# NilFoundation/vote-saver-protocol

Hardware: AMD Instinct MI355X
Metric: G1 MSM points/sec at 2^20 (Groth16 prover hot path) (higher is better)
Workload: dtype u32; 1 GPU; 2^20-point BLS12-381 G1 Pippenger MSM per GPU, PLAIN bases k_i*G (no table of window multiples; the library's 28-bit-limb copy keeps phi(P) = (beta x, y) beside every P for the endomorphism split), uniform scalars, bases and scalars resident in HBM; N ranks = one 2^20*N-point MSM sharded by contiguous chunk, RCCL all-gather of Jacobian partial sums + fold; points_per_gpu=1048576, window_bits=16, windows=8, endomorphism_split=True, msms_in_flight=4, bases_precomputed_window_multiples=False, bases_memory_bytes_per_point=352

## Files before the change

### vote_saver_protocol_amd/csrc/common.h

```cpp
#pragma once
#include <hip/hip_runtime.h>
#include <stdint.h>
#include <stdio.h>
#include <string.h>
#include <functional>
#include <initializer_list>
#include <map>
#include <string>
#include <vector>

#include "../../include/vsp.h"
#include <atomic>
#include <mutex>
#include <thread>
#include "curve.h"
#include "point_decode.h"
#include "saver_ct.h"
#include "saver_rerand.h"

struct vsp_ctx;
namespace vsp {

struct Affine28; struct Affine28x2;
template <int N> struct Group;
// ... 62 lines not shown

struct MsmGeom {
    unsigned c;
    unsigned W;
    unsigned B;
    unsigned q0, q1, q2;
    unsigned T;
    size_t n;
    size_t G;
    unsigned Wr;
    unsigned single;
    uint32_t idx_stride, idx_first;
    unsigned sbits;
    unsigned lb;
    unsigned fold;
    unsigned bd;
    unsigned K, Wk;
    size_t kstride;
};
struct MsmPre { size_t stride; size_t first; unsigned c; const void *table28; bool glv; };

struct MsmWork {
    static constexpr size_t PINNED_BYTES = 256 * 1024;
    bool inited = false, own_stream = false, active = false, empty = false;
    bool dimbits = false;
    hipStream_t stream = nullptr;
    hipStream_t own = nullptr;
    hipEvent_t ev0 = nullptr, ev1 = nullptr, done = nullptr, plan_ready = nullptr;
    DevBuf cnt, off, cursor, nsub, suboff, blocksum, sorted, heavy, counters, digits, blockhist, partbucket, perm, sizehist;
    DevBuf buckets, partials, dims, winres, medium, redo;
    DevBuf buckets28, partials28;
    DevBuf pairs_a, pairs_b, ms_h1, ms_h1s, ms_h2, ms_h2s;
    DevBuf tmp_sorted, tmp_lo, off_hi, cnt_hi;
    DevBuf glv_scalars;
    bool glv = false;
    void *h_pinned = nullptr;
    size_t pinned_cap = 0;
    static constexpr unsigned REC_RING = 4;
    void *h_rec = nullptr; hipEvent_t rec_ev[REC_RING] = {nullptr, nullptr, nullptr, nullptr}; unsigned rec_idx = 0;
    void *h_census = nullptr;
    hipEvent_t census_done = nullptr;
    bool census_pending = false; size_t census_n = 0; const void *census_scalars = nullptr;
    bool check_pending = false;
    size_t neff_cache_n = 0, neff_cache = 0;
    MsmGeom g;
    size_t n = 0, n_eff = 0;
};
static constexpr unsigned VSP_MSM_SLOTS = 6;
struct MsmTuning { long window_bits = 0, split = 0, dimbits = -1; };
struct MsmRequest {
    const void *bases = nullptr;
    const Fr *scalars = nullptr;
    size_t n = 0;
    int plan_from = -1;
    bool dense = false;
    bool plan_only = false;
    const MsmPre *pre = nullptr;
    const void *table28 = nullptr;
    bool glv = false;
    unsigned batch = 0;
    size_t stride = 0;
    const MsmTuning *tuning = nullptr;
    MsmRequest(const Fr *scalars_ = nullptr, size_t n_ = 0) : scalars(scalars_), n(n_) {}
};
struct MsmLaunch {
    MsmRequest rq;
    hipStream_t st;
    const MsmWork *plan_from;
    const void *table28;
    const Fr *scalars; size_t n;
    long sort_mode;
    MsmTuning tune;
    bool fused_split, fused_scans, dimbits;
    size_t M, Smax;
    unsigned per_w, nblk, gblk, ablk;
};
static constexpr unsigned MSM_THREADS = 256;
static constexpr unsigned SZ_BINS = 1024;
__device__ __forceinline__ uint32_t part_len(uint32_t s, uint32_t parts) { return (s + parts - 1) / parts; }

enum NttPath { NTT_AUTO, NTT_FR29, NTT_FR32 };
struct NttRequest {
    const Fr *in[3] = {nullptr, nullptr, nullptr};
    Fr *out[3] = {nullptr, nullptr, nullptr};
    unsigned count = 1;
    size_t in_stride = 0, out_stride = 0;
    const Fr *fuse_b = nullptr, *fuse_c = nullptr;
    unsigned log_m = 0;
    int inverse = 0;
    const uint64_t *coset_g = nullptr;
    const HFr *extra_scale = nullptr;
    NttPath path = NTT_AUTO;
    NttRequest(Fr *d_a, unsigned log_m_, int inverse_ = 0, const uint64_t *coset_g_ = nullptr, const HFr *extra_scale_ = nullptr)
        : log_m(log_m_), inverse(inverse_), coset_g(coset_g_), extra_scale(extra_scale_) { in[0] = d_a; out[0] = d_a; }
};

}

struct vsp_ctx {
    int device = 0;
    hipStream_t stream = nullptr;
    hipStream_t own_stream = nullptr;
    hipStream_t prove_streams[2] = {nullptr, nullptr};
    hipEvent_t ev0 = nullptr, ev1 = nullptr, ev_aux = nullptr;
    std::string err;
    std::map<std::string, double> stats;
// ... 418 lines not shown
```

### vote_saver_protocol_amd/csrc/msm_impl.inc

```
#include "common.h"
#include "lane_view.h"
#include "fp28.h"
#if VSP_MSM_GROUP == 1
#include "accum28_asm_gfx950.h"
#endif


namespace vsp {
namespace {

#if VSP_MSM_GROUP == 1
static constexpr uint32_t GLV_BETA_MONT[12] = {0x8671f071u, 0xcd03c9e4u, 0x1fcda5d2u, 0x5dab2246u, 0xd3851b95u, 0x587042afu, 0x01bacb9eu, 0x8eb60ebeu, 0x83d050d2u, 0x03f97d6eu, 0x54638741u, 0x18f02065u};
#else
static constexpr uint32_t GLV_BETA_MONT[12] = {0x798a64e8u, 0x30f1361bu, 0x7ece5a2au, 0xf3b8ddabu, 0xc61577f7u, 0x16a8ca3au, 0x74fd029bu, 0xc26a2ff8u, 0x60701c6eu, 0x3636b766u, 0x241b6160u, 0x051ba4abu};
#endif
__device__ __forceinline__ Fp glv_beta() { Fp b; for (int i = 0; i < 12; i++) b.l[i] = GLV_BETA_MONT[i]; return b; }
__device__ __forceinline__ void glv_apply(Fp &x) { x = mul(x, glv_beta()); }
__device__ __forceinline__ void glv_apply(Fp2 &x) { Fp b = glv_beta(); x.c0 = mul(x.c0, b); x.c1 = mul(x.c1, b); }
__device__ __forceinline__ void glv_apply(Fp2L &x) { x.v = mul(x.v, glv_beta()); }

template <class F> struct AccumWaves { static constexpr unsigned W = 2; };
template <class F>
__device__ __forceinline__ XYZZ<typename LaneView<F>::E> accumulate_part(const Affine<F> *__restrict__ bases, const uint32_t *__restrict__ sorted, const uint32_t *__restrict__ off,
                                                const uint32_t *__restrict__ suboff, const uint32_t *__restrict__ part_bucket, uint32_t q,
// ... 750 lines not shown
    const long wide = opt(ctx, "msm_wide_windows", 1);
    if (c == 16 && wide && !glv && n >= ((size_t)1 << 20)) c = 17;
    if (c >= 16 && wide && n >= ((size_t)1 << 23)) {
        double best = 0; int bc = 16;
        for (int k = 16; k <= 23; k++) {
            const double W = glv ? (double)((128 + k - 1) / k) : (double)((255 % k == 0 ? 254 : 255) / k + 1);
            const double cost = (double)n * W * (k > 16 ? 0.87 : 1.0) + W * (double)((size_t)1 << (k - 1)) * 4.1;
            if (k == 16 || cost < best) { best = cost; bc = k; }
        }
        c = bc;
    }
    return (unsigned)c;
}

#if VSP_MSM_GROUP == 1
using F28 = Fp28; using Row28 = Affine28;
#else
using F28 = Fp2x28; using Row28 = Affine28x2;
#endif

template <class F> static int msm_geometry(vsp_ctx *ctx, MsmWork &wk, MsmLaunch &L, MsmGeom &g, size_t &n_eff) {
    const MsmPre *pre = L.rq.pre; const bool glv = L.rq.glv; const size_t n = L.rq.n; const unsigned batch = L.rq.batch;
    const uint32_t imul = glv ? 2u : 1u;
    n_eff = n;
    if (L.plan_from) {
        g = L.plan_from->g; n_eff = L.plan_from->n_eff;
        if (L.plan_from->n != n) return set_error(ctx, VSP_ERR_ARG, "msm: shared plan of a different size");
        if ((g.single != 0) != (pre != nullptr) || (pre && (g.idx_stride != pre->stride * imul || g.idx_first != pre->first * imul || g.c != pre->c)))
            return set_error(ctx, VSP_ERR_ARG, "msm: shared plan needs bases precomputed alike");
    } else {
        VSP_TRY(ensure_w(ctx, L.st, wk.counters, 64));
        wk.check_pending = false;
        if (!L.rq.dense) {
            if (!(wk.census_pending && wk.census_n == n && wk.census_scalars == (const void *)L.rq.scalars)) VSP_TRY(msm_census(ctx, wk, L.rq.scalars, n, nullptr, batch, L.rq.stride));
            wk.check_pending = true;
            if (n >= 4096) {
                if (wk.neff_cache_n == n && !opt(ctx, "msm_census_sync", 0)) n_eff = wk.neff_cache;
                else {
                    VSP_HIP(hipEventSynchronize(wk.census_done));
                    uint32_t h_cnt = *(volatile uint32_t *)wk.h_census / batch;
                    n_eff = h_cnt < 256 ? 256 : h_cnt;
                }
            }
        }
        wk.census_pending = false;
        if (glv) n_eff *= 2;
        g.c = pre ? pre->c : pick_window_bits(ctx, L.tune.window_bits, n_eff, glv);
        g.sbits = glv ? 128u : 255u;
        g.fold = (!glv && opt(ctx, "msm_fold", 1) && 255u % g.c == 0u) ? 1u : 0u;
        if (batch > 1 && g.c > 16) g.c = 16;
        if (batch > 1 && g.c < 7) g.c = 7;
        g.Wk = glv ? (128u + g.c - 1) / g.c : (g.fold ? 254u / g.c + 1 : g.sbits / g.c + 1);
        g.K = batch; g.kstride = batch > 1 ? L.rq.stride : 0;
        g.W = g.Wk * g.K;
        g.B = 1u << (g.c - 1);
        g.lb = g.c > 16 ? g.c - 16 : 0u;
        g.n = glv ? 2 * n : n;
        g.single = pre ? 1u : 0u; g.idx_stride = pre ? (uint32_t)(pre->stride * imul) : 0u; g.idx_first = pre ? (uint32_t)(pre->first * imul) : 0u;
        g.Wr = pre ? g.K : g.W;
        g.G = (size_t)g.Wr * g.B;
        const long t = L.tune.split;
        if (pre) {
            size_t est = n_eff * g.W / ((size_t)1 << 18);
            unsigned T = 16; while (T < est && T < (1u << 20)) T <<= 1;
            if (T >= 64) T = T / 8 * 7;
            g.T = t > 0 ? (unsigned)t : T;
            if ((size_t)g.Wk * pre->stride * imul >= ((size_t)1 << 31)) return set_error(ctx, VSP_ERR_UNSUPPORTED, "msm: precomputed table too large to index");
        } else {
            size_t mean = n_eff / g.B + 1;
            size_t T = mean * 4 < 128 ? 128 : mean * 4;
// ... 80 lines not shown
                           g.G, g.T, buckets28, partials28, redo + 1, redo);
        VSP_HIP(hipEventRecord(wk.ev1, st));
        hipLaunchKernelGGL(HIP_KERNEL_NAME(k_accum_redo<F>), dim3(L.ablk < 64 ? L.ablk : 64), dim3(MSM_THREADS), 0, st, bases, (const uint32_t *)pl->sorted.p,
                           (const uint32_t *)pl->off.p, (const uint32_t *)pl->suboff.p, (const uint32_t *)pl->partbucket.p, buckets, partials,
                           (const uint32_t *)(redo + 1), (const uint32_t *)redo, L.rq.glv, buckets28, partials28);
        VSP_LAUNCH_CHECK();
        return launch_tail<F28>(ctx, st, pl, g, L.dimbits, buckets28, partials28, (XYZZ<F28> *)wk.dims.p, winres, (XYZZ<F> *)wk.h_pinned);
    }
    VSP_HIP(hipEventRecord(wk.ev0, st));
    hipLaunchKernelGGL(HIP_KERNEL_NAME(k_accum<F>), dim3(L.ablk * LaneView<F>::LANES), dim3(MSM_THREADS), 0, st, bases, (const uint32_t *)pl->sorted.p,
                       (const uint32_t *)pl->off.p, (const uint32_t *)pl->suboff.p, (const uint32_t *)pl->perm.p, (const uint32_t *)pl->partbucket.p,
                       g.G, g.T, buckets, partials);
    VSP_HIP(hipEventRecord(wk.ev1, st));
    VSP_LAUNCH_CHECK();
    return launch_tail<F>(ctx, st, pl, g, L.dimbits, buckets, partials, (XYZZ<F> *)wk.dims.p, winres, (XYZZ<F> *)wk.h_pinned);
}

template <class F>
static int msm_launch(vsp_ctx *ctx, MsmWork &wk, const MsmRequest &rq, const MsmWork *plan_from) {
    const size_t n = rq.n;
    wk.active = false; wk.n = n;
    if (n == 0) { wk.active = true; wk.empty = true; wk.g.K = rq.batch ? rq.batch : 1; return VSP_OK; }
    wk.empty = false;
    const unsigned batch = rq.batch ? rq.batch : 1;
    if (batch > 1 && rq.plan_only) return set_error(ctx, VSP_ERR_UNSUPPORTED, "msm: a batch plans and accumulates in one launch");
    if (batch > 1 && plan_from && (plan_from->g.K != batch || plan_from->g.kstride != rq.stride || !plan_from->active || plan_from->empty))
        return set_error(ctx, VSP_ERR_ARG, "msm: shared plan of another batch");
    MsmLaunch L{};
    L.rq = rq; L.rq.batch = batch; L.st = wk.stream; L.scalars = rq.scalars; L.n = n;
    L.table28 = rq.pre ? rq.pre->table28 : rq.table28;
    L.rq.glv = rq.glv && (rq.pre ? rq.pre->glv && rq.pre->table28 : rq.table28 != nullptr);
    if (n >= ((size_t)1 << (L.rq.glv ? 30 : 31))) return set_error(ctx, VSP_ERR_UNSUPPORTED, "msm: n >= 2^31");
    L.plan_from = plan_from && plan_from->glv == L.rq.glv ? plan_from : nullptr;
    wk.glv = L.rq.glv;
    L.sort_mode = opt(ctx, "msm_sort", 0);
    L.tune = rq.tuning ? *rq.tuning : MsmTuning{opt(ctx, "msm_window_bits", 0), opt(ctx, "msm_split", 0), opt(ctx, "msm_dimbits", -1)};
    MsmGeom g; size_t n_eff = n;
    VSP_TRY(msm_geometry<F>(ctx, wk, L, g, n_eff));
    wk.g = g; wk.n_eff = n_eff;
    VSP_TRY(msm_split_scalars(ctx, wk, L, g));
    VSP_TRY(msm_buffers<F>(ctx, wk, L, g));
    if (L.plan_from) VSP_HIP(hipStreamWaitEvent(L.st, L.plan_from->plan_ready, 0));
    else { VSP_TRY(msm_digit_sort(ctx, wk, L, g)); VSP_TRY(msm_bucket_plan(ctx, wk, L, g)); }
    if (rq.plan_only) return VSP_OK;
    VSP_TRY(msm_accumulate<F>(ctx, wk, L, g));
    VSP_HIP(hipEventRecord(wk.done, L.st));
    wk.active = true;
    return VSP_OK;
}

template <class F, class HF> static void msm_fold(const MsmWork &wk, XYZZ<HF> *out);
template <class F, class HF>
static int msm_finish_wait(vsp_ctx *ctx, MsmWork &wk, unsigned out_count, bool *empty);
template <class F, class HF>
static int msm_finish(vsp_ctx *ctx, MsmWork &wk, XYZZ<HF> *out, unsigned out_count = 1) {
    for (unsigned k = 0; k < out_count; k++) out[k] = XYZZ<HF>::inf();
    bool empty = false;
    VSP_TRY((msm_finish_wait<F, HF>(ctx, wk, out_count, &empty)));
    if (!empty) msm_fold<F, HF>(wk, out);
    return VSP_OK;
}
template <class F, class HF>
static int msm_finish_wait(vsp_ctx *ctx, MsmWork &wk, unsigned out_count, bool *empty) {
    static_assert(sizeof(F) == sizeof(HF), "host/device field layouts must match");
    *empty = true;
    if (!wk.active) return set_error(ctx, VSP_ERR_ARG, "msm: finish without launch");
    wk.active = false;
    if (wk.empty) return VSP_OK;
    *empty = false;
    if (wk.g.K != out_count) return set_error(ctx, VSP_ERR_ARG, "msm: finish asks for another number of results than the launch's batch");
    VSP_HIP(hipEventSynchronize(wk.done));
    const MsmGeom &g = wk.g;
#ifdef VSP_DEBUG_DUMP
    if (const char *dir = getenv("VSP_DEBUG_DUMP_DIR")) {
        if (FILE *f = fopen((std::string(dir) + "/winres.bin").c_str(), "wb")) { fwrite(wk.h_pinned, 1, (size_t)g.Wr * (wk.dimbits ? DIMBITS_STRIDE : 4) * sizeof(XYZZ<HF>), f); fclose(f); }
        const unsigned per_w = dims_per_w(g);
        std::vector<char> hb(g.G * sizeof(XYZZ<F>)), hd((size_t)g.Wr * per_w * sizeof(XYZZ<F>));
        if (wk.buckets.p && wk.dims.p && hipMemcpy(hb.data(), wk.buckets.p, hb.size(), hipMemcpyDeviceToHost) == hipSuccess &&
            hipMemcpy(hd.data(), wk.dims.p, hd.size(), hipMemcpyDeviceToHost) == hipSuccess) {
            std::string d(dir);
            if (FILE *f = fopen((d + "/buckets.bin").c_str(), "wb")) { fwrite(hb.data(), 1, hb.size(), f); fclose(f); }
            if (FILE *f = fopen((d + "/dims.bin").c_str(), "wb")) { fwrite(hd.data(), 1, hd.size(), f); fclose(f); }
            if (FILE *f = fopen((d + "/geom.txt").c_str(), "w")) { fprintf(f, "%u %u %u %u %u %u %u %zu\n", g.c, g.W, g.Wr, g.B, g.q0, g.q1, g.q2, sizeof(XYZZ<F>)); fclose(f); }
        }
    }
#endif
    if (wk.check_pending) {
        wk.check_pending = false;
        VSP_HIP(hipEventSynchronize(wk.census_done));
        const volatile uint32_t *hc = (const volatile uint32_t *)wk.h_census;
        if (wk.n >= 4096) { const uint32_t c0 = hc[0] / (wk.g.K ? wk.g.K : 1u); wk.neff_cache_n = wk.n; wk.neff_cache = c0 < 256 ? 256 : c0; }
        if (hc[2]) return set_error(ctx, VSP_ERR_ARG, "msm: a scalar is not canonical (>= r)");
    }
    float ms = 0.f;
    if (hipEventElapsedTime(&ms, wk.ev0, wk.ev1) == hipSuccess) {
        ctx->stats["msm_accum_ms"] += ms;
        ctx->stats["msm_accum_launches"] += 1;
    }
    ctx->stats["msm_calls"] += 1;
    ctx->stats["msm_n_eff"] = (double)wk.n_eff;
    ctx->stats["msm_window_bits"] = g.c;
    ctx->stats["msm_windows"] = g.W;
    ctx->stats["msm_bucket_sets"] = g.Wr;
    ctx->stats["msm_split"] = g.T;
    ctx->stats["msm_endomorphism_split"] = wk.glv ? 1 : 0;
    if (opt(ctx, "msm_debug_counts", 0) && wk.counters.p && wk.suboff.p) {
        uint32_t c4[4] = {0, 0, 0, 0}, parts = 0;
        if (hipMemcpy(c4, wk.counters.p, sizeof c4, hipMemcpyDeviceToHost) == hipSuccess &&
            hipMemcpy(&parts, (const uint32_t *)wk.suboff.p + g.G, 4, hipMemcpyDeviceToHost) == hipSuccess) {
            ctx->stats["msm_heavy_buckets"] = c4[0]; ctx->stats["msm_medium_buckets"] = c4[2]; ctx->stats["msm_parts"] = parts;
            ctx->stats["msm_buckets"] = (double)g.G;
        }
    }
    return VSP_OK;
}
template <class F, class HF> static void msm_fold(const MsmWork &wk, XYZZ<HF> *out) {
    const MsmGeom &g = wk.g;
    const XYZZ<HF> *wr = (const XYZZ<HF> *)wk.h_pinned;
    const unsigned per = g.single ? 1u : (g.K > 1 ? g.Wk : g.Wr);
// ... 111 lines not shown
```

### vote_saver_protocol_amd/csrc/msm_sort.hip

```cpp
#include "common.h"

namespace vsp {
namespace {


__device__ __forceinline__ uint32_t scalar_bits(const uint32_t *k, unsigned pos, unsigned c) {
    unsigned limb = pos >> 5, sh = pos & 31;
    if (limb >= 8) return 0;
    uint64_t v = k[limb];
    if (limb + 1 < 8) v |= (uint64_t)k[limb + 1] << 32;
    return (uint32_t)(v >> sh) & ((1u << c) - 1u);
}

__device__ __forceinline__ uint32_t load_scalar(const Fr *scalars, size_t i, const MsmGeom &g, uint32_t (&k)[8]) {
    const uint32_t *p = scalars[i].l;
#pragma unroll
    for (int j = 0; j < 8; j++) k[j] = p[j];
    if (g.sbits == 128u) return k[7] >> 31;
    if (!g.fold) return 0u;
    uint32_t d[8], borrow = 0;
#pragma unroll
    for (int j = 0; j < 8; j++) {
        const uint64_t t = (uint64_t)FrP32::MOD[j] - k[j] - borrow;
        d[j] = (uint32_t)t; borrow = (uint32_t)(t >> 63);
// ... 150 lines not shown
    if (threadIdx.x == 0 && bad) atomicOr(&counters[3], 1u);
}

#ifndef VSP_CS_ATTR
#define VSP_CS_ATTR
#endif
#ifndef VSP_CS_UNROLL
#define VSP_CS_UNROLL
#endif
#ifndef VSP_CS_THREADS
#define VSP_CS_THREADS 1024
#endif
static constexpr unsigned CS_THREADS = VSP_CS_THREADS;
static constexpr unsigned CS_MLP = 8;
static constexpr uint16_t DIGIT_NONE = 0xFFFFu;

__global__ __launch_bounds__(256) void k_digits(const Fr *scalars, MsmGeom g, uint16_t *digits, uint8_t *flips) {
    size_t i = (size_t)blockIdx.x * blockDim.x + threadIdx.x;
    if (i >= g.n) return;
    const unsigned kb = blockIdx.y;
    scalars += (size_t)kb * g.kstride;
    uint32_t k[8];
    const uint32_t flip = load_scalar(scalars, i, g, k);
    uint32_t carry = 0;
    if (g.sbits == 128u || g.fold) flips[(size_t)kb * g.n + i] = (uint8_t)flip;
    for (unsigned w = 0; w < g.Wk; w++) {
        uint32_t raw = scalar_bits(k, w * g.c, g.c) + carry;
        uint32_t mag; uint32_t neg;
        if (raw > g.B) { mag = (1u << g.c) - raw; neg = 1; carry = 1; }
        else { mag = raw; neg = 0; carry = 0; }
        digits[(size_t)(kb * g.Wk + w) * g.n + i] = mag ? (uint16_t)((mag - 1) | (neg << 15)) : DIGIT_NONE;
    }
}
__global__ __launch_bounds__(256) void k_glv_digits(const Fr *scalars, size_t n_orig, MsmGeom g, uint16_t *digits, uint8_t *flips) {
    size_t i = (size_t)blockIdx.x * blockDim.x + threadIdx.x;
    if (i >= n_orig) return;
    const unsigned kb = blockIdx.y;
    scalars += (size_t)kb * g.kstride;
    flips += (size_t)kb * g.n;
    uint32_t k[8], m[2][8]; bool neg[2];
    load_scalar_words(scalars, i, k);
    {
        uint32_t m1[4], m2[4];
        glv_split_scalar(k, m1, neg[0], m2, neg[1]);
#pragma unroll
        for (int j = 0; j < 8; j++) { m[0][j] = j < 4 ? m1[j] : 0u; m[1][j] = j < 4 ? m2[j] : 0u; }
    }
    reinterpret_cast<uint16_t *>(flips)[i] = (uint16_t)((neg[0] ? 1u : 0u) | (neg[1] ? 0x100u : 0u));
    uint32_t carry[2] = {0, 0};
    uint32_t *d32 = reinterpret_cast<uint32_t *>(digits);
    for (unsigned w = 0; w < g.Wk; w++) {
        uint32_t pair = 0;
#pragma unroll
        for (int b = 0; b < 2; b++) {
            const uint32_t raw = scalar_bits(m[b], w * g.c, g.c) + carry[b];
            uint32_t mag, ng;
            if (raw > g.B) { mag = (1u << g.c) - raw; ng = 1; carry[b] = 1; }
            else { mag = raw; ng = 0; carry[b] = 0; }
            const uint32_t d = mag ? ((mag - 1) | (ng << 15)) : (uint32_t)DIGIT_NONE;
            pair |= d << (16 * b);
        }
        d32[((size_t)(kb * g.Wk + w) * g.n) / 2 + i] = pair;
    }
}

__global__ __launch_bounds__(256) void k_digits_wide(const Fr *scalars, MsmGeom g, uint16_t *hi, uint8_t *lo) {
    size_t i = (size_t)blockIdx.x * blockDim.x + threadIdx.x;
    if (i >= g.n) return;
    uint32_t k[8];
    const uint32_t flip = load_scalar(scalars, i, g, k);
    uint32_t carry = 0;
    for (unsigned w = 0; w < g.W; w++) {
        uint32_t raw = scalar_bits(k, w * g.c, g.c) + carry;
// ... 78 lines not shown
    for (size_t base = i0; base < i1; base += (size_t)CS_MLP * CS_THREADS) {
        uint16_t dd[CS_MLP]; uint8_t ff[CS_MLP];
#pragma unroll
        for (unsigned j = 0; j < CS_MLP; j++) {
            const size_t i = base + (size_t)j * CS_THREADS + threadIdx.x;
            dd[j] = i < i1 ? dw[i] : DIGIT_NONE;
            ff[j] = (use_flips && i < i1) ? flips[(size_t)(w / g.Wk) * g.n + i] : (uint8_t)0;
        }
#pragma unroll
        for (unsigned j = 0; j < CS_MLP; j++) {
            const size_t i = base + (size_t)j * CS_THREADS + threadIdx.x;
            const uint16_t d = dd[j];
            const bool valid = d != DIGIT_NONE;
            const uint32_t key = d & 0x7FFFu;
            const unsigned long long act = __ballot(valid);
            if (act) {
                const int lead = __ffsll((long long)act) - 1;
                const uint32_t lkey = (uint32_t)__shfl((int)key, lead, 64);
                const bool same = valid && key == lkey;
                const unsigned long long grp = __ballot(same);
                const unsigned lane = threadIdx.x & 63u;
                uint32_t pos = 0;
                if (same && (int)lane == lead) pos = atomicAdd(&lds_cur[lkey], (uint32_t)__popcll(grp));
                pos = (uint32_t)__shfl((int)pos, lead, 64) + (uint32_t)__popcll(grp & ((1ull << lane) - 1ull));
                if (valid && !same) pos = atomicAdd(&lds_cur[key], 1u);
                if (valid) {
                    uint32_t sign;
                    if (lo_in) { const uint8_t l = lo_in[(size_t)w * g.n + i]; sign = l >> 7; lo_out[pos] = l & 0x7Fu; }
                    else sign = (uint32_t)(d >> 15) ^ (uint32_t)ff[j];
                    sorted[pos] = entry_of(g, w, i) | (sign << 31);
                }
            }
        }
    }
}

__global__ __launch_bounds__(256) void k_segment_sort(const uint32_t *__restrict__ tmp_sorted, const uint8_t *__restrict__ tmp_lo, const uint32_t *__restrict__ off_hi,
                                                     size_t segments, unsigned lb, uint32_t *cnt, uint32_t *off, uint32_t *sorted) {
    __shared__ uint32_t sh[4][128];
    const unsigned wave = threadIdx.x >> 6, lane = threadIdx.x & 63u;
    uint32_t *c = sh[wave];
    const unsigned nb = 1u << lb;
    const unsigned long long below = (1ull << lane) - 1ull;
    for (size_t s = (size_t)blockIdx.x * 4 + wave; s < segments; s += (size_t)gridDim.x * 4) {
        const uint32_t a = off_hi[s], b = off_hi[s + 1];
        c[lane] = 0; c[lane + 64] = 0;
        __builtin_amdgcn_wave_barrier();
        for (uint32_t j0 = a; j0 < b; j0 += 64) {
            const uint32_t j = j0 + lane;
            const bool valid = j < b;
            const uint32_t l = valid ? tmp_lo[j] : 0u;
            unsigned long long peers = __ballot(valid);
            for (unsigned k = 0; k < lb; k++) { const bool bit = (l >> k) & 1u; const unsigned long long m = __ballot(valid && bit); peers &= bit ? m : ~m; }
            if (valid && (int)lane == __ffsll((long long)peers) - 1) atomicAdd(&c[l], (uint32_t)__popcll(peers));
        }
        __builtin_amdgcn_wave_barrier();
        const uint32_t c0 = c[lane], c1 = c[lane + 64];
        uint32_t i0 = c0, i1 = c1;
        for (int d = 1; d < 64; d <<= 1) { uint32_t x0 = __shfl_up(i0, d, 64), x1 = __shfl_up(i1, d, 64); if ((int)lane >= d) { i0 += x0; i1 += x1; } }
        const uint32_t tot0 = __shfl(i0, 63, 64);
        const uint32_t e0 = a + i0 - c0, e1 = a + tot0 + i1 - c1;
        const size_t g0 = (s << lb) + lane;
        if (lane < nb) { cnt[g0] = c0; off[g0] = e0; }
        if (lane + 64 < nb) { cnt[g0 + 64] = c1; off[g0 + 64] = e1; }
        __builtin_amdgcn_wave_barrier();
        c[lane] = e0; c[lane + 64] = e1;
// ... 540 lines not shown
    VSP_TRY(ensure_w(ctx, st, wk.off_hi, (gh.G + 1) * 4));
    VSP_TRY(ensure_w(ctx, st, wk.tmp_sorted, L.M * 4));
    VSP_TRY(ensure_w(ctx, st, wk.tmp_lo, L.M));
    uint16_t *hi = (uint16_t *)wk.digits.p; uint8_t *lo = (uint8_t *)(hi + (size_t)g.W * n);
    uint32_t *blockhist = (uint32_t *)wk.blockhist.p, *cnt_hi = (uint32_t *)wk.cnt_hi.p, *off_hi = (uint32_t *)wk.off_hi.p;
    const size_t lds_bytes = (size_t)gh.B * sizeof(uint32_t);
    VSP_TRY(lds_sort_attrs(ctx));
    hipLaunchKernelGGL(k_digits_wide, dim3(L.nblk), dim3(MSM_THREADS), 0, st, L.scalars, g, hi, lo);
    hipLaunchKernelGGL(k_count_lds, dim3(nchunks * g.W), dim3(CS_THREADS), lds_bytes, st, (const uint16_t *)hi, gh, nchunks, chunk_len, blockhist);
    hipLaunchKernelGGL(k_chunk_prefix, dim3((unsigned)((gh.G + MSM_THREADS - 1) / MSM_THREADS)), dim3(MSM_THREADS), 0, st, blockhist, g.single ? nchunks * g.W : nchunks, gh.G, cnt_hi, (uint32_t *)nullptr, gh.G);
    VSP_LAUNCH_CHECK();
    VSP_TRY(exclusive_scan_w(ctx, wk, cnt_hi, gh.G, off_hi, nullptr));
    hipLaunchKernelGGL(k_scatter_lds, dim3(nchunks * g.W), dim3(CS_THREADS), lds_bytes, st, (const uint16_t *)hi, (const uint8_t *)nullptr, gh, nchunks, chunk_len,
                       (const uint32_t *)blockhist, (const uint32_t *)off_hi, (uint32_t *)wk.tmp_sorted.p, (const uint8_t *)lo, (uint8_t *)wk.tmp_lo.p);
    { size_t wg = (gh.G + 3) / 4; if (wg > 65536) wg = 65536;
      hipLaunchKernelGGL(k_segment_sort, dim3((unsigned)wg), dim3(256), 0, st, (const uint32_t *)wk.tmp_sorted.p, (const uint8_t *)wk.tmp_lo.p, (const uint32_t *)off_hi,
                         gh.G, g.lb, (uint32_t *)wk.cnt.p, (uint32_t *)wk.off.p, (uint32_t *)wk.sorted.p); }
    VSP_LAUNCH_CHECK();
    return VSP_OK;
}

static int msm_sort_lds(vsp_ctx *ctx, MsmWork &wk, const MsmLaunch &L, const MsmGeom &g) {
    const hipStream_t st = L.st; const size_t n = L.n;
    uint32_t *cnt = (uint32_t *)wk.cnt.p, *off = (uint32_t *)wk.off.p;
    const bool batch_single = g.single && g.K > 1;
    const unsigned nchunks = batch_single ? 1u : lds_chunks(g, n);
    const size_t chunk_len = (n + nchunks - 1) / nchunks;
    VSP_TRY(ensure_w(ctx, st, wk.digits, (size_t)g.W * n * sizeof(uint16_t) + (size_t)g.K * n));
    VSP_TRY(ensure_w(ctx, st, wk.blockhist, (size_t)nchunks * g.W * g.B * sizeof(uint32_t)));
    uint16_t *digits = (uint16_t *)wk.digits.p; uint32_t *blockhist = (uint32_t *)wk.blockhist.p;
    uint8_t *flips = (uint8_t *)(digits + (size_t)g.W * n);
    const size_t lds_bytes = (size_t)g.B * sizeof(uint32_t);
    VSP_TRY(lds_sort_attrs(ctx));
    if (L.fused_split) hipLaunchKernelGGL(k_glv_digits, dim3((unsigned)((L.rq.n + MSM_THREADS - 1) / MSM_THREADS), g.K), dim3(MSM_THREADS), 0, st, L.rq.scalars, L.rq.n, g, digits, flips);
    else hipLaunchKernelGGL(k_digits, dim3(L.nblk, g.K), dim3(MSM_THREADS), 0, st, L.scalars, g, digits, flips);
    hipLaunchKernelGGL(k_count_lds, dim3(nchunks * g.W), dim3(CS_THREADS), lds_bytes, st, (const uint16_t *)digits, g, nchunks, chunk_len, blockhist);
    VSP_TRY(ensure_w(ctx, st, wk.blocksum, ((size_t)L.gblk + 2) * sizeof(uint32_t)));
    uint32_t *tilesum = (uint32_t *)wk.blocksum.p;
    hipLaunchKernelGGL(k_chunk_prefix, dim3(L.gblk), dim3(MSM_THREADS), 0, st, blockhist, batch_single ? g.Wk : (g.single ? nchunks * g.W : nchunks), g.G, cnt,
                       L.fused_scans ? tilesum : (uint32_t *)nullptr, batch_single ? (size_t)g.B : g.G);
    VSP_LAUNCH_CHECK();
    if (L.fused_scans) hipLaunchKernelGGL(k_scan_tiles256, dim3(L.gblk), dim3(MSM_THREADS), 0, st, (const uint32_t *)cnt, g.G, (const uint32_t *)tilesum, off, (uint32_t *)nullptr);
    else VSP_TRY(exclusive_scan_w(ctx, wk, cnt, g.G, off, nullptr));
    hipLaunchKernelGGL(k_scatter_lds, dim3(nchunks * g.W), dim3(CS_THREADS), lds_bytes, st, (const uint16_t *)digits, (const uint8_t *)flips, g, nchunks, chunk_len,
                       (const uint32_t *)blockhist, (const uint32_t *)off, (uint32_t *)wk.sorted.p, (const uint8_t *)nullptr, (uint8_t *)nullptr);
    VSP_LAUNCH_CHECK();
    return VSP_OK;
}

int msm_digit_sort(vsp_ctx *ctx, MsmWork &wk, MsmLaunch &L, const MsmGeom &g) {
    VSP_HIP(hipMemsetAsync(wk.counters.p, 0, 64, L.st));
    L.fused_scans = opt(ctx, "msm_fused_scans", 1) && L.gblk <= 4096;
    const size_t n = L.n;
    const bool staged = g.K == 1 && g.c >= 12 && g.c <= 23 && n >= 4096 && L.sort_mode != 1 && (L.sort_mode == 2 || (g.c >= 17 && n >= ((size_t)1 << 20)));
    if (staged) return msm_sort_staged(ctx, wk, L, g);
    if (g.c > 16 && n >= ((size_t)1 << 15)) return msm_sort_wide(ctx, wk, L, g);
    if (g.c <= 16 && (n >= ((size_t)1 << 15) || g.K > 1)) return msm_sort_lds(ctx, wk, L, g);
    uint32_t *cnt = (uint32_t *)wk.cnt.p, *cursor = (uint32_t *)wk.cursor.p;
    VSP_HIP(hipMemsetAsync(cnt, 0, (g.G + 1) * 4, L.st));
    hipLaunchKernelGGL(k_count, dim3(L.nblk), dim3(MSM_THREADS), 0, L.st, L.scalars, g, cnt);
    VSP_LAUNCH_CHECK();
    VSP_TRY(exclusive_scan_w(ctx, wk, cnt, g.G, (uint32_t *)wk.off.p, cursor));
    hipLaunchKernelGGL(k_scatter, dim3(L.nblk), dim3(MSM_THREADS), 0, L.st, L.scalars, g, cursor, (uint32_t *)wk.sorted.p);
    VSP_LAUNCH_CHECK();
    return VSP_OK;
}

int msm_bucket_plan(vsp_ctx *ctx, MsmWork &wk, const MsmLaunch &L, const MsmGeom &g) {
    const hipStream_t st = L.st;
    const uint32_t *cnt = (const uint32_t *)wk.cnt.p;
    uint32_t *nsub = (uint32_t *)wk.nsub.p, *suboff = (uint32_t *)wk.suboff.p;
    VSP_TRY(ensure_w(ctx, st, wk.blocksum, ((size_t)L.gblk + 2) * sizeof(uint32_t)));
    uint32_t *tilesum = (uint32_t *)wk.blocksum.p;
    uint32_t *size_hist = (uint32_t *)wk.sizehist.p, *bin_cursor = size_hist + SZ_BINS;
    uint32_t *redo0 = nullptr;
    if (!L.rq.plan_only && L.table28) { VSP_TRY(ensure_w(ctx, st, wk.redo, (L.Smax + 1) * sizeof(uint32_t))); redo0 = (uint32_t *)wk.redo.p; }
    hipLaunchKernelGGL(k_plan, dim3(L.gblk), dim3(MSM_THREADS), 0, st, cnt, g.G, g.T, nsub, (uint32_t *)wk.heavy.p, (uint32_t *)wk.medium.p, (uint32_t *)wk.counters.p,
                       L.fused_scans ? tilesum : (uint32_t *)nullptr, size_hist, 2u * SZ_BINS, redo0);
    VSP_LAUNCH_CHECK();
    if (L.fused_scans) hipLaunchKernelGGL(k_scan_tiles256, dim3(L.gblk), dim3(MSM_THREADS), 0, st, (const uint32_t *)nsub, g.G, (const uint32_t *)tilesum, suboff, (uint32_t *)nullptr);
    else VSP_TRY(exclusive_scan_w(ctx, wk, nsub, g.G, suboff, nullptr));
    uint32_t *part_bucket = (uint32_t *)wk.partbucket.p, *perm = (uint32_t *)wk.perm.p;
    hipLaunchKernelGGL(k_partinfo, dim3(L.ablk), dim3(256), 0, st, cnt, (const uint32_t *)suboff, g.G, g.T, part_bucket, size_hist);
    hipLaunchKernelGGL(k_binscan, dim3(1), dim3(SZ_BINS), 0, st, (const uint32_t *)size_hist, bin_cursor);
    hipLaunchKernelGGL(k_partsort, dim3(L.ablk), dim3(256), 0, st, cnt, (const uint32_t *)suboff, (const uint32_t *)part_bucket, g.G, g.T, bin_cursor, perm);
    VSP_LAUNCH_CHECK();
    VSP_HIP(hipEventRecord(wk.plan_ready, st));
    return VSP_OK;
// ... 8 lines not shown
}
int msm_slot_census(vsp_ctx *ctx, unsigned slot_id, const Fr *d_scalars, size_t n) {
    if (slot_id >= VSP_MSM_SLOTS) return set_error(ctx, VSP_ERR_ARG, "msm: bad slot");
    VSP_TRY(work_init(ctx, slot(ctx, slot_id), slot_id == 0 ? ctx->stream : nullptr));
    if (n == 0) return VSP_OK;
    return msm_census(ctx, slot(ctx, slot_id), d_scalars, n, ctx->stream);
}
int msm_slot_stream(vsp_ctx *ctx, unsigned slot_id, hipStream_t *out) {
    if (slot_id >= VSP_MSM_SLOTS) return set_error(ctx, VSP_ERR_ARG, "msm: bad slot");
    VSP_TRY(work_init(ctx, slot(ctx, slot_id), slot_id == 0 ? ctx->stream : nullptr));
    *out = slot(ctx, slot_id).stream;
    return VSP_OK;
}
int msm_slot_use_stream(vsp_ctx *ctx, unsigned slot_id, hipStream_t stream_or_null) {
    if (slot_id == 0 || slot_id >= VSP_MSM_SLOTS) return set_error(ctx, VSP_ERR_ARG, "msm: bad slot");
    MsmWork &wk = slot(ctx, slot_id);
    wk.stream = stream_or_null;
    return stream_or_null ? work_init(ctx, wk, nullptr) : VSP_OK;
}
void msm_drain_slots(vsp_ctx *ctx) {
    for (unsigned i = 0; i < VSP_MSM_SLOTS; i++) {
        MsmWork &w = ctx->msm_work[i];
        if (!w.inited) continue;
        if (w.stream) hipStreamSynchronize(w.stream);
        w.active = false; w.check_pending = false; w.census_pending = false;
    }
    hipStreamSynchronize(ctx->stream);
    hipGetLastError();
}
void msm_free_slots(vsp_ctx *ctx) {
    for (unsigned i = 0; i < VSP_MSM_SLOTS; i++) {
        MsmWork &w = ctx->msm_work[i];
        DevBuf *bufs[] = {&w.cnt, &w.off, &w.cursor, &w.nsub, &w.suboff, &w.blocksum, &w.sorted, &w.heavy, &w.counters, &w.digits, &w.blockhist,
                          &w.partbucket, &w.perm, &w.sizehist, &w.buckets, &w.partials, &w.dims, &w.winres, &w.medium, &w.redo, &w.glv_scalars, &w.buckets28, &w.partials28, &w.tmp_sorted, &w.tmp_lo, &w.off_hi, &w.cnt_hi, &w.pairs_a, &w.pairs_b, &w.ms_h1, &w.ms_h1s, &w.ms_h2, &w.ms_h2s};
        for (DevBuf *b : bufs) { if (b->p) hipFree(b->p); b->p = nullptr; b->cap = 0; }
        if (w.inited) {
            hipEventDestroy(w.ev0); hipEventDestroy(w.ev1); hipEventDestroy(w.done); hipEventDestroy(w.plan_ready);
            hipHostFree(w.h_pinned); hipHostFree(w.h_census); hipEventDestroy(w.census_done);
            hipHostFree(w.h_rec); for (unsigned k = 0; k < MsmWork::REC_RING; k++) hipEventDestroy(w.rec_ev[k]);
            if (w.own_stream && w.own) hipStreamDestroy(w.own);
            w.own = nullptr; w.stream = nullptr; w.own_stream = false;
            w.inited = false;
        }
    }
}

}
```

Before: 375.4 million points/s.

## Add tiled two-level digit sort and fuse scalar census into GLV digit kernel

Adds a new tiled sort path for 13–16-bit windows. Per-tile coarse-bin histograms are scanned globally and used to place packed records by coarse bin, and a per-bin kernel then does a fine 8-bit LDS counting sort that writes cnt/off/sorted directly. This replaces the LDS chunk count/scatter sort for 2^17..2^23 points. It also defers the scalar census when a cached n_eff exists and folds its nonzero count and range-check into the GLV digit kernel through wave ballots, saving a separate pass over the scalars. The cost is extra record and tile-histogram buffers plus one extra global pass through the records.

```diff
diff --git a/vote_saver_protocol_amd/csrc/common.h b/vote_saver_protocol_amd/csrc/common.h
--- a/vote_saver_protocol_amd/csrc/common.h
+++ b/vote_saver_protocol_amd/csrc/common.h
@@ -118,8 +118,10 @@
     DevBuf buckets28, partials28;
     DevBuf pairs_a, pairs_b, ms_h1, ms_h1s, ms_h2, ms_h2s;
     DevBuf tmp_sorted, tmp_lo, off_hi, cnt_hi;
+    DevBuf tilehist, tileoff, records;
     DevBuf glv_scalars;
     bool glv = false;
+    bool sort_tiled = false, census_fused = false;
     void *h_pinned = nullptr;
     size_t pinned_cap = 0;
     static constexpr unsigned REC_RING = 4;
@@ -158,6 +160,7 @@
     long sort_mode;
     MsmTuning tune;
     bool fused_split, fused_scans, dimbits;
+    bool census_deferred;
     size_t M, Smax;
     unsigned per_w, nblk, gblk, ablk;
 };
diff --git a/vote_saver_protocol_amd/csrc/msm_impl.inc b/vote_saver_protocol_amd/csrc/msm_impl.inc
--- a/vote_saver_protocol_amd/csrc/msm_impl.inc
+++ b/vote_saver_protocol_amd/csrc/msm_impl.inc
@@ -806,10 +806,14 @@
         VSP_TRY(ensure_w(ctx, L.st, wk.counters, 64));
         wk.check_pending = false;
         if (!L.rq.dense) {
-            if (!(wk.census_pending && wk.census_n == n && wk.census_scalars == (const void *)L.rq.scalars)) VSP_TRY(msm_census(ctx, wk, L.rq.scalars, n, nullptr, batch, L.rq.stride));
+            const bool cached = n >= 4096 && wk.neff_cache_n == n && !opt(ctx, "msm_census_sync", 0);
+            if (!(wk.census_pending && wk.census_n == n && wk.census_scalars == (const void *)L.rq.scalars)) {
+                if (cached && batch == 1 && !L.rq.pre) L.census_deferred = true;
+                else VSP_TRY(msm_census(ctx, wk, L.rq.scalars, n, nullptr, batch, L.rq.stride));
+            }
             wk.check_pending = true;
             if (n >= 4096) {
-                if (wk.neff_cache_n == n && !opt(ctx, "msm_census_sync", 0)) n_eff = wk.neff_cache;
+                if (cached) n_eff = wk.neff_cache;
                 else {
                     VSP_HIP(hipEventSynchronize(wk.census_done));
                     uint32_t h_cnt = *(volatile uint32_t *)wk.h_census / batch;
@@ -956,7 +960,7 @@
     L.rq.glv = rq.glv && (rq.pre ? rq.pre->glv && rq.pre->table28 : rq.table28 != nullptr);
     if (n >= ((size_t)1 << (L.rq.glv ? 30 : 31))) return set_error(ctx, VSP_ERR_UNSUPPORTED, "msm: n >= 2^31");
     L.plan_from = plan_from && plan_from->glv == L.rq.glv ? plan_from : nullptr;
-    wk.glv = L.rq.glv;
+    wk.glv = L.rq.glv; wk.sort_tiled = wk.census_fused = false;
     L.sort_mode = opt(ctx, "msm_sort", 0);
     L.tune = rq.tuning ? *rq.tuning : MsmTuning{opt(ctx, "msm_window_bits", 0), opt(ctx, "msm_split", 0), opt(ctx, "msm_dimbits", -1)};
     MsmGeom g; size_t n_eff = n;
@@ -1009,6 +1013,8 @@
         }
     }
 #endif
+    ctx->stats["msm_sort_tiled"] = wk.sort_tiled ? 1 : 0;
+    ctx->stats["msm_census_fused"] = wk.census_fused ? 1 : 0;
     if (wk.check_pending) {
         wk.check_pending = false;
         VSP_HIP(hipEventSynchronize(wk.census_done));
diff --git a/vote_saver_protocol_amd/csrc/msm_sort.hip b/vote_saver_protocol_amd/csrc/msm_sort.hip
--- a/vote_saver_protocol_amd/csrc/msm_sort.hip
+++ b/vote_saver_protocol_amd/csrc/msm_sort.hip
@@ -206,13 +206,27 @@
         digits[(size_t)(kb * g.Wk + w) * g.n + i] = mag ? (uint16_t)((mag - 1) | (neg << 15)) : DIGIT_NONE;
     }
 }
-__global__ __launch_bounds__(256) void k_glv_digits(const Fr *scalars, size_t n_orig, MsmGeom g, uint16_t *digits, uint8_t *flips) {
+__global__ __launch_bounds__(256) void k_glv_digits(const Fr *scalars, size_t n_orig, MsmGeom g, uint16_t *digits, uint8_t *flips, uint32_t *census) {
     size_t i = (size_t)blockIdx.x * blockDim.x + threadIdx.x;
-    if (i >= n_orig) return;
     const unsigned kb = blockIdx.y;
     scalars += (size_t)kb * g.kstride;
     flips += (size_t)kb * g.n;
     uint32_t k[8], m[2][8]; bool neg[2];
+    if (census) {
+        const bool live = i < n_orig;
+        bool counted = false, bad = false;
+        if (live) {
+            load_scalar_words(scalars, i, k);
+            counted = (k[1] | k[2] | k[3] | k[4] | k[5] | k[6] | k[7]) != 0 || k[0] > 1;
+            bad = k[7] >= 0x73eda753u && !scalar_below_r(make_uint4(k[0], k[1], k[2], k[3]), make_uint4(k[4], k[5], k[6], k[7]));
+        }
+        const unsigned long long cm = __ballot(counted), bm = __ballot(bad);
+        if ((threadIdx.x & 63u) == 0) {
+            if (cm) atomicAdd(&census[1], (uint32_t)__popcll(cm));
+            if (bm) atomicOr(&census[3], 1u);
+        }
+    }
+    if (i >= n_orig) return;
     load_scalar_words(scalars, i, k);
     {
         uint32_t m1[4], m2[4];
@@ -357,6 +371,148 @@
                 }
             }
         }
+    }
+}
+
+static constexpr unsigned TS_THREADS = 256, TS_TILE = 8192, TS_PIECE = 2048, TS_MLP = 8;
+static constexpr unsigned TS_MIN_LOG = 17, TS_MAX_LOG = 23;
+
+__device__ __forceinline__ uint32_t ts_scan(uint32_t v, uint32_t *sh, uint32_t *total) {
+    const unsigned lane = threadIdx.x & 63u, wave = threadIdx.x >> 6;
+    uint32_t incl = v;
+    for (int d = 1; d < 64; d <<= 1) { const uint32_t x = __shfl_up(incl, d, 64); if ((int)lane >= d) incl += x; }
+    __syncthreads();
+    if (lane == 63) sh[wave] = incl;
+    __syncthreads();
+    uint32_t base = 0, tot = 0;
+#pragma unroll
+    for (unsigned k = 0; k < TS_THREADS / 64; k++) { const uint32_t s = sh[k]; if (k < wave) base += s; tot += s; }
+    if (total) *total = tot;
+    return base + incl - v;
+}
+__device__ __forceinline__ uint32_t ts_take(uint32_t *ctr, bool valid, uint32_t key) {
+    const unsigned long long act = __ballot(valid);
+    if (!act) return 0u;
+    const unsigned lane = threadIdx.x & 63u;
+    const int lead = __ffsll((long long)act) - 1;
+    const uint32_t lkey = (uint32_t)__shfl((int)key, lead, 64);
+    const bool same = valid && key == lkey;
+    const unsigned long long grp = __ballot(same);
+    uint32_t pos = 0;
+    if (same && (int)lane == lead) pos = atomicAdd(&ctr[lkey], (uint32_t)__popcll(grp));
+    pos = (uint32_t)__shfl((int)pos, lead, 64) + (uint32_t)__popcll(grp & ((1ull << lane) - 1ull));
+    if (valid && !same) pos = atomicAdd(&ctr[key], 1u);
+    return pos;
+}
+
+__global__ __launch_bounds__(TS_THREADS) void k_tile_hist(const uint16_t *__restrict__ digits, MsmGeom g, unsigned ntiles, uint32_t *__restrict__ tilehist) {
+    __shared__ uint32_t h[128];
+    const unsigned tile = blockIdx.x % ntiles, w = blockIdx.x / ntiles, nbins = 1u << (g.c - 9);
+    if (threadIdx.x < 128) h[threadIdx.x] = 0;
+    __syncthreads();
+    const size_t i0 = (size_t)tile * TS_TILE, i1 = i0 + TS_TILE < g.n ? i0 + TS_TILE : g.n;
+    const uint16_t *dw = digits + (size_t)w * g.n;
+    for (size_t base = i0; base < i1; base += (size_t)TS_MLP * TS_THREADS) {
+        uint16_t dd[TS_MLP];
+#pragma unroll
+        for (unsigned j = 0; j < TS_MLP; j++) { const size_t i = base + (size_t)j * TS_THREADS + threadIdx.x; dd[j] = i < i1 ? dw[i] : DIGIT_NONE; }
+#pragma unroll
+        for (unsigned j = 0; j < TS_MLP; j++) ts_take(h, dd[j] != DIGIT_NONE, (dd[j] & 0x7FFFu) >> 8);
+    }
+    __syncthreads();
+    if (threadIdx.x < nbins) tilehist[((size_t)w * nbins + threadIdx.x) * ntiles + tile] = h[threadIdx.x];
+}
+
+__global__ __launch_bounds__(TS_THREADS) void k_tile_place(const uint16_t *__restrict__ digits, const uint8_t *__restrict__ flips, MsmGeom g, unsigned ntiles,
+                                                          const uint32_t *__restrict__ tilehist, const uint32_t *__restrict__ tileoff, uint32_t *__restrict__ records) {
+    __shared__ uint32_t buf[TS_TILE];
+    __shared__ uint32_t toff[128], cur[128], gstart[128], sh[TS_THREADS / 64], count_sh;
+    const unsigned tile = blockIdx.x % ntiles, w = blockIdx.x / ntiles, nbins = 1u << (g.c - 9), tid = threadIdx.x;
+    {
+        const size_t slot = ((size_t)w * nbins + tid) * ntiles + tile;
+        const uint32_t v = tid < nbins ? tilehist[slot] : 0u;
+        uint32_t tot;
+        const uint32_t ex = ts_scan(v, sh, &tot);
+        if (tid < nbins) { toff[tid] = ex; cur[tid] = ex; gstart[tid] = tileoff[slot]; }
+        if (tid == 0) count_sh = tot;
+    }
+    __syncthreads();
+    const size_t i0 = (size_t)tile * TS_TILE, i1 = i0 + TS_TILE < g.n ? i0 + TS_TILE : g.n;
+    const uint16_t *dw = digits + (size_t)w * g.n;
+    const bool use_flips = g.sbits == 128u || g.fold;
+    for (unsigned base = 0; base < TS_TILE && i0 + base < i1; base += TS_MLP * TS_THREADS) {
+        uint16_t dd[TS_MLP]; uint8_t ff[TS_MLP];
+#pragma unroll
+        for (unsigned j = 0; j < TS_MLP; j++) {
+            const size_t i = i0 + base + j * TS_THREADS + tid;
+            dd[j] = i < i1 ? dw[i] : DIGIT_NONE;
+            ff[j] = (use_flips && i < i1) ? flips[i] : (uint8_t)0;
+        }
+#pragma unroll
+        for (unsigned j = 0; j < TS_MLP; j++) {
+            const uint32_t d = dd[j], key = d & 0x7FFFu;
+            const bool valid = d != DIGIT_NONE;
+            const uint32_t pos = ts_take(cur, valid, key >> 8);
+            if (valid) buf[pos] = (base + j * TS_THREADS + tid) | (((d >> 15) ^ (uint32_t)ff[j]) << 13) | (key << 14);
+        }
+    }
+    __syncthreads();
+    const unsigned count = count_sh;
+    for (unsigned k = tid; k < count; k += TS_THREADS) {
+        const uint32_t x = buf[k], key = x >> 14, bin = key >> 8;
+        records[(size_t)gstart[bin] + (k - toff[bin])] = ((uint32_t)(i0 + (x & (TS_TILE - 1u))) << 9) | (((x >> 13) & 1u) << 8) | (key & 0xFFu);
+    }
+}
+
+__global__ __launch_bounds__(TS_THREADS) void k_bin_sort(const uint32_t *__restrict__ records, const uint32_t *__restrict__ tileoff, MsmGeom g, unsigned ntiles,
+                                                        uint32_t *__restrict__ cnt, uint32_t *__restrict__ off, uint32_t *__restrict__ sorted) {
+    __shared__ uint32_t buf[TS_PIECE];
+    __shared__ uint32_t h[256], cur[256], poff[256], sh[TS_THREADS / 64];
+    const unsigned slot = blockIdx.x, tid = threadIdx.x;
+    const uint32_t a = tileoff[(size_t)slot * ntiles], b = tileoff[((size_t)slot + 1) * ntiles];
+    h[tid] = 0;
+    __syncthreads();
+    for (uint32_t base = a; base < b; base += TS_MLP * TS_THREADS) {
+        uint32_t rr[TS_MLP];
+#pragma unroll
+        for (unsigned j = 0; j < TS_MLP; j++) { const uint32_t i = base + j * TS_THREADS + tid; rr[j] = i < b ? records[i] : 0xFFFFFFFFu; }
+#pragma unroll
+        for (unsigned j = 0; j < TS_MLP; j++) ts_take(h, base + j * TS_THREADS + tid < b, rr[j] & 0xFFu);
+    }
+    __syncthreads();
+    {
+        const uint32_t c0 = h[tid];
+        const uint32_t ex = ts_scan(c0, sh, nullptr);
+        const size_t gi = (size_t)slot * 256 + tid;
+        cnt[gi] = c0; off[gi] = a + ex;
+        cur[tid] = a + ex;
+        if (slot == gridDim.x - 1 && tid == 0) off[g.G] = b;
+        h[tid] = 0;
+    }
+    __syncthreads();
+    constexpr unsigned PER = TS_PIECE / TS_THREADS;
+    for (uint32_t base = a; base < b; base += TS_PIECE) {
+        uint32_t rr[PER], rk[PER];
+#pragma unroll
+        for (unsigned j = 0; j < PER; j++) { const uint32_t i = base + j * TS_THREADS + tid; rr[j] = i < b ? records[i] : 0xFFFFFFFFu; }
+#pragma unroll
+        for (unsigned j = 0; j < PER; j++) rk[j] = ts_take(h, base + j * TS_THREADS + tid < b, rr[j] & 0xFFu);
+        __syncthreads();
+        const uint32_t pc = h[tid];
+        uint32_t tot;
+        const uint32_t pex = ts_scan(pc, sh, &tot);
+        poff[tid] = pex;
+        __syncthreads();
+#pragma unroll
+        for (unsigned j = 0; j < PER; j++) if (base + j * TS_THREADS + tid < b) buf[poff[rr[j] & 0xFFu] + rk[j]] = rr[j];
+        __syncthreads();
+        for (unsigned k = tid; k < tot; k += TS_THREADS) {
+            const uint32_t x = buf[k], bk = x & 0xFFu;
+            sorted[(size_t)cur[bk] + (k - poff[bk])] = (x >> 9) | (((x >> 8) & 1u) << 31);
+        }
+        __syncthreads();
+        cur[tid] += pc; h[tid] = 0;
+        __syncthreads();
     }
 }
 
@@ -963,7 +1119,7 @@
     uint8_t *flips = (uint8_t *)(digits + (size_t)g.W * n);
     const size_t lds_bytes = (size_t)g.B * sizeof(uint32_t);
     VSP_TRY(lds_sort_attrs(ctx));
-    if (L.fused_split) hipLaunchKernelGGL(k_glv_digits, dim3((unsigned)((L.rq.n + MSM_THREADS - 1) / MSM_THREADS), g.K), dim3(MSM_THREADS), 0, st, L.rq.scalars, L.rq.n, g, digits, flips);
+    if (L.fused_split) hipLaunchKernelGGL(k_glv_digits, dim3((unsigned)((L.rq.n + MSM_THREADS - 1) / MSM_THREADS), g.K), dim3(MSM_THREADS), 0, st, L.rq.scalars, L.rq.n, g, digits, flips, (uint32_t *)nullptr);
     else hipLaunchKernelGGL(k_digits, dim3(L.nblk, g.K), dim3(MSM_THREADS), 0, st, L.scalars, g, digits, flips);
     hipLaunchKernelGGL(k_count_lds, dim3(nchunks * g.W), dim3(CS_THREADS), lds_bytes, st, (const uint16_t *)digits, g, nchunks, chunk_len, blockhist);
     VSP_TRY(ensure_w(ctx, st, wk.blocksum, ((size_t)L.gblk + 2) * sizeof(uint32_t)));
@@ -979,12 +1135,49 @@
     return VSP_OK;
 }
 
+static bool sort_tiles_apply(const vsp_ctx *ctx, const MsmLaunch &L, const MsmGeom &g) {
+    return opt(ctx, "msm_sort_tiles", 1) && !g.single && g.K == 1 && g.c >= 13 && g.c <= 16 && L.n >= ((size_t)1 << TS_MIN_LOG) && L.n <= ((size_t)1 << TS_MAX_LOG);
+}
+static int msm_sort_tiled(vsp_ctx *ctx, MsmWork &wk, const MsmLaunch &L, const MsmGeom &g, bool census) {
+    const hipStream_t st = L.st; const size_t n = L.n;
+    const unsigned ntiles = (unsigned)((n + TS_TILE - 1) / TS_TILE), nbins = 1u << (g.c - 9);
+    const size_t H = (size_t)g.W * nbins * ntiles;
+    VSP_TRY(ensure_w(ctx, st, wk.digits, (size_t)g.W * n * sizeof(uint16_t) + n));
+    VSP_TRY(ensure_w(ctx, st, wk.tilehist, (H + 1) * 4)); VSP_TRY(ensure_w(ctx, st, wk.tileoff, (H + 1) * 4));
+    VSP_TRY(ensure_w(ctx, st, wk.records, L.M * 4));
+    uint16_t *digits = (uint16_t *)wk.digits.p; uint8_t *flips = (uint8_t *)(digits + (size_t)g.W * n);
+    uint32_t *tilehist = (uint32_t *)wk.tilehist.p, *tileoff = (uint32_t *)wk.tileoff.p, *records = (uint32_t *)wk.records.p;
+    if (L.fused_split) {
+        uint32_t *counters = (uint32_t *)wk.counters.p;
+        hipLaunchKernelGGL(k_glv_digits, dim3((unsigned)((L.rq.n + MSM_THREADS - 1) / MSM_THREADS), 1), dim3(MSM_THREADS), 0, st, L.rq.scalars, L.rq.n, g, digits, flips, census ? counters : (uint32_t *)nullptr);
+        VSP_LAUNCH_CHECK();
+        if (census) {
+            VSP_HIP(hipMemcpyAsync(wk.h_census, counters + 1, 12, hipMemcpyDeviceToHost, st));
+            VSP_HIP(hipEventRecord(wk.census_done, st));
+        }
+    } else hipLaunchKernelGGL(k_digits, dim3(L.nblk, 1), dim3(MSM_THREADS), 0, st, L.scalars, g, digits, flips);
+    hipLaunchKernelGGL(k_tile_hist, dim3(g.W * ntiles), dim3(TS_THREADS), 0, st, (const uint16_t *)digits, g, ntiles, tilehist);
+    VSP_LAUNCH_CHECK();
+    VSP_TRY(exclusive_scan_w(ctx, wk, tilehist, H, tileoff, nullptr));
+    hipLaunchKernelGGL(k_tile_place, dim3(g.W * ntiles), dim3(TS_THREADS), 0, st, (const uint16_t *)digits, (const uint8_t *)flips, g, ntiles,
+                       (const uint32_t *)tilehist, (const uint32_t *)tileoff, records);
+    hipLaunchKernelGGL(k_bin_sort, dim3(g.W * nbins), dim3(TS_THREADS), 0, st, (const uint32_t *)records, (const uint32_t *)tileoff, g, ntiles,
+                       (uint32_t *)wk.cnt.p, (uint32_t *)wk.off.p, (uint32_t *)wk.sorted.p);
+    VSP_LAUNCH_CHECK();
+    return VSP_OK;
+}
+
 int msm_digit_sort(vsp_ctx *ctx, MsmWork &wk, MsmLaunch &L, const MsmGeom &g) {
     VSP_HIP(hipMemsetAsync(wk.counters.p, 0, 64, L.st));
+    const bool staged_first = g.K == 1 && g.c >= 12 && g.c <= 23 && L.n >= 4096 && L.sort_mode != 1 && (L.sort_mode == 2 || (g.c >= 17 && L.n >= ((size_t)1 << 20)));
+    const bool tiled = !staged_first && sort_tiles_apply(ctx, L, g);
+    const bool fused_census = L.census_deferred && tiled && L.fused_split;
+    wk.sort_tiled = tiled; wk.census_fused = fused_census;
+    if (L.census_deferred && !fused_census) { VSP_TRY(msm_census(ctx, wk, L.rq.scalars, L.rq.n, nullptr, L.rq.batch, L.rq.stride)); wk.census_pending = false; }
     L.fused_scans = opt(ctx, "msm_fused_scans", 1) && L.gblk <= 4096;
     const size_t n = L.n;
-    const bool staged = g.K == 1 && g.c >= 12 && g.c <= 23 && n >= 4096 && L.sort_mode != 1 && (L.sort_mode == 2 || (g.c >= 17 && n >= ((size_t)1 << 20)));
-    if (staged) return msm_sort_staged(ctx, wk, L, g);
+    if (staged_first) return msm_sort_staged(ctx, wk, L, g);
+    if (tiled) return msm_sort_tiled(ctx, wk, L, g, fused_census);
     if (g.c > 16 && n >= ((size_t)1 << 15)) return msm_sort_wide(ctx, wk, L, g);
     if (g.c <= 16 && (n >= ((size_t)1 << 15) || g.K > 1)) return msm_sort_lds(ctx, wk, L, g);
     uint32_t *cnt = (uint32_t *)wk.cnt.p, *cursor = (uint32_t *)wk.cursor.p;
@@ -1059,7 +1252,7 @@
     for (unsigned i = 0; i < VSP_MSM_SLOTS; i++) {
         MsmWork &w = ctx->msm_work[i];
         DevBuf *bufs[] = {&w.cnt, &w.off, &w.cursor, &w.nsub, &w.suboff, &w.blocksum, &w.sorted, &w.heavy, &w.counters, &w.digits, &w.blockhist,
-                          &w.partbucket, &w.perm, &w.sizehist, &w.buckets, &w.partials, &w.dims, &w.winres, &w.medium, &w.redo, &w.glv_scalars, &w.buckets28, &w.partials28, &w.tmp_sorted, &w.tmp_lo, &w.off_hi, &w.cnt_hi, &w.pairs_a, &w.pairs_b, &w.ms_h1, &w.ms_h1s, &w.ms_h2, &w.ms_h2s};
+                          &w.partbucket, &w.perm, &w.sizehist, &w.buckets, &w.partials, &w.dims, &w.winres, &w.medium, &w.redo, &w.glv_scalars, &w.buckets28, &w.partials28, &w.tmp_sorted, &w.tmp_lo, &w.off_hi, &w.cnt_hi, &w.pairs_a, &w.pairs_b, &w.ms_h1, &w.ms_h1s, &w.ms_h2, &w.ms_h2s, &w.tilehist, &w.tileoff, &w.records};
         for (DevBuf *b : bufs) { if (b->p) hipFree(b->p); b->p = nullptr; b->cap = 0; }
         if (w.inited) {
             hipEventDestroy(w.ev0); hipEventDestroy(w.ev1); hipEventDestroy(w.done); hipEventDestroy(w.plan_ready);
```

After: 371.6 million points/s. 1.0% lower.
